# Gwzwpxz/HDSDP

Measured on AMD Instinct MI355X. Metric: IPM iterations/sec (Schur build+factor+solve), n=2000 m=2000 dense SDP, higher is better.
Workload: dtype f64

## Files before the change

### hdsdp_amd/csrc/chol.h

```cpp
#pragma once
#include "hdm_common.h"
#include <vector>

struct HdmChol {
    int n = 0, npad = 0, nblk = 0;
    HdmBuf<double> L;
    HdmBuf<double> Linv;
    HdmBuf<double> Dinv;
    HdmBuf<double> Z;
    HdmBuf<double> Zd;
    HdmBuf<double> vec;
    HdmBuf<int> info_dev;
    bool factored = false, have_inv = false;
    bool logdet_ok = false;
    double logdet_val = 0.0;
    HdmBuf<int> flow_flags;
    HdmPinned<int> flow_err;
    int flow_epoch = 0;
    bool flow_ok = true, flow_pending = false;
    int flow_cap = -1;
    std::vector<double> host_stage;
    std::vector<int> env_first, env_colh;
    HdmBuf<int> env_dev;
    HdmBuf<double> sgn;
    HdmBuf<int> sinfo_dev;

    int init(int n);
    int set_envelope(const int *first_blockcol_of_blockrow);
    int load_host(const double *A, long lda, hipStream_t s);
    int load_device(const double *A, long lda, hipStream_t s);
    int finish_load(hipStream_t s);
    int factor(hipStream_t s, int *info_host);
    int invert_factor(hipStream_t s);
    int set_reverse_inverse(hipStream_t s);
    int factor_signed(hipStream_t s, int *info_host, int *nneg_host);
    int reverse_signs(double *sig_dev, hipStream_t s);
    int get_diag(double *diag_host, hipStream_t s);
    int solve_device(double *b_dev, double *x_dev, int nrhs, long ldv, int which, hipStream_t s);
    int solve_host(const double *rhs, double *sol, int nrhs, int which, hipStream_t s);
    bool flow_gave_up();
    int inverse_full(double *out_dev, long ldo, hipStream_t s);
};

int hdm_potrf_sweep_configure();
int hdm_potrf_sweep_batched(double *tiles, const int *diag_tile, const int *cols, int ncols, double *Winv, int *info, int m, hipStream_t s,
                            double *sgn = nullptr);

void hdm_flow_set_shared_device(int on);
bool hdm_flow_shared_device();
double hdm_diag_block_probe(int variant, int reps, hipStream_t s);
```

### hdsdp_amd/csrc/chol.hip

```cpp
#include "hdm_common.h"
#include "chol.h"
#include "sweep128.h"
#include <algorithm>
#include <atomic>
#include <cstring>

#define NB 128

#define PB 32
#define LDW 98
__device__ __forceinline__ double hdm_readlane_f64(double v, int lane) {
    int lo = __double2loint(v), hi = __double2hiint(v);
    lo = __builtin_amdgcn_readlane(lo, lane);
    hi = __builtin_amdgcn_readlane(hi, lane);
    return __hiloint2double(hi, lo);
}

typedef double hdm_c4 __attribute__((ext_vector_type(4)));

template <int NT>
__device__ __forceinline__ void hdm_lds_mm(double *pc, int crs, int ccs, const double *pa, int ars, int acs, const double *pb,
                                           int brs, int bcs, int M, int N, int K, double alpha, int accumulate, int k_by_row,
                                           int lower_only, int wave, int lane, double *gout, long gld) {
    const int l15 = lane & 15, lq = lane >> 4;
    const int mt = M >> 4, nt = (N >> 4) / NT, units = mt * nt;
    for (int u = wave; u < units; u += 4) {
        const int ti = u / nt, tj = (u % nt) * NT;
        if (lower_only && tj > ti) continue;
        hdm_c4 acc[NT];
#pragma unroll
        for (int q = 0; q < NT; ++q) acc[q] = (hdm_c4){0.0, 0.0, 0.0, 0.0};
        const int kend = k_by_row ? min(K, (ti + 1) * 16) : K;
        const double *qa = pa + (ti * 16 + l15) * ars + lq * acs;
        const double *qb = pb + lq * brs + (tj * 16 + l15) * bcs;
        for (int k0 = 0; k0 < kend; k0 += 4) {
            const double av = qa[k0 * acs];
#pragma unroll
            for (int q = 0; q < NT; ++q) acc[q] = __builtin_amdgcn_mfma_f64_16x16x4f64(qb[k0 * brs + q * 16 * bcs], av, acc[q], 0, 0, 0);
        }
#pragma unroll
        for (int q = 0; q < NT; ++q)
#pragma unroll
            for (int r = 0; r < 4; ++r) {
                const int m = ti * 16 + l15, n = (tj + q) * 16 + lq + 4 * r;
                double *c = pc + m * crs + n * ccs;
                const double v = (accumulate ? *c : 0.0) + alpha * acc[q][r];
                *c = v;
                if (gout) gout[m + (long) n * gld] = v;
            }
    }
}

__global__ __launch_bounds__(256) void hdm_potrf_diag_kernel(double *__restrict__ A, long ld, double *__restrict__ Dinv,
                                                              int *__restrict__ info, int col0) {
    extern __shared__ __attribute__((aligned(16))) double sm[];
    double *a = sm;
    double *w = sm + NB * NB;
    const int tid = threadIdx.x;
    for (int e0 = tid; e0 < NB * NB; e0 += 256 * 16) {
        double v[16];
#pragma unroll
        for (int q = 0; q < 16; ++q) {
            const int e = e0 + q * 256;
            v[q] = A[(e & (NB - 1)) + (long) (e >> 7) * ld];
        }
#pragma unroll
        for (int q = 0; q < 16; ++q) {
            const int e = e0 + q * 256;
            a[e] = ((e & (NB - 1)) >= (e >> 7)) ? v[q] : 0.0;
        }
    }
    __syncthreads();

    for (int p = 0; p < NB / PB; ++p) {
        const int c0 = p * PB;
        if (tid < 64) {
            const int l = tid & 31;
            double *blk = a + c0 + c0 * NB;
            double row[PB], rinv[PB];
#pragma unroll
            for (int k = 0; k < PB; ++k) row[k] = blk[l + k * NB];
            int bad = 0;
#pragma unroll
            for (int j = 0; j < PB; ++j) {
                double d = hdm_readlane_f64(row[j], j);
                if (!(d > 0.0)) {
                    if (!bad) bad = j + 1;
                    d = 1.0;
                }
                const double piv = sqrt(d);
                double ri = 1.0 / piv;
                asm volatile("" : "+v"(ri));
                rinv[j] = ri;
                row[j] = (l == j) ? piv : row[j] * ri;
#pragma unroll
                for (int k = j + 1; k < PB; ++k) row[k] -= row[j] * hdm_readlane_f64(row[j], k);
                __builtin_amdgcn_sched_barrier(0);
            }
            if (bad && tid == 0) atomicCAS(info, 0, col0 + c0 + bad);
            if (tid < PB) {
#pragma unroll
                for (int k = 0; k < PB; ++k)
                    if (k <= l) A[(c0 + l) + (long) (c0 + k) * ld] = row[k];
            }
#pragma unroll
            for (int k = 0; k < PB; ++k) asm volatile("" : "+v"(row[k]));
            double x[PB];
#pragma unroll
            for (int i = 0; i < PB; ++i) {
                double sacc = (l == i) ? 1.0 : 0.0;
#pragma unroll
                for (int k = 0; k < i; ++k) sacc -= hdm_readlane_f64(row[k], i) * x[k];
                x[i] = (l <= i) ? sacc * rinv[i] : 0.0;
                __builtin_amdgcn_sched_barrier(0);
            }
            if (tid < PB) {
#pragma unroll
                for (int i = 0; i < PB; ++i) blk[i + l * NB] = x[i];
            }
        }
        __syncthreads();
        const int t0 = c0 + PB, nr = NB - t0;
        if (nr <= 0) break;
        const int wave = tid >> 6, lane = tid & 63;
        hdm_lds_mm<2>(a + t0 + c0 * NB, 1, NB, a + t0 + c0 * NB, 1, NB, a + c0 + c0 * NB, NB, 1, nr, PB, PB, 1.0, 0, 0, 0, wave,
                      lane, A + t0 + (long) c0 * ld, ld);
        __syncthreads();
        hdm_lds_mm<1>(a + t0 + t0 * NB, 1, NB, a + t0 + c0 * NB, 1, NB, a + t0 + c0 * NB, NB, 1, nr, nr, PB, -1.0, 1, 0, 1, wave,
                      lane, nullptr, 0);
        __syncthreads();
    }
    {
        const int wave = tid >> 6, lane = tid & 63;
        for (int j = NB / PB - 2; j >= 0; --j) {
            const int c0 = j * PB, r0 = c0 + PB, nr = NB - r0;
            hdm_lds_mm<2>(w, 1, LDW, a + r0 + c0 * NB, 1, NB, a + c0 + c0 * NB, 1, NB, nr, PB, PB, 1.0, 0, 0, 0, wave, lane,
                          nullptr, 0);
            __syncthreads();
            hdm_lds_mm<2>(a + r0 + c0 * NB, 1, NB, a + r0 + r0 * NB, 1, NB, w, 1, LDW, nr, PB, nr, -1.0, 0, 1, 0, wave, lane,
                          nullptr, 0);
            __syncthreads();
        }
    }
    for (int e = tid; e < NB * NB; e += 256) Dinv[e] = a[e];
}

#define DIAG_SWEEP_LDS_DOUBLES (SMALL_P * (SMALL_P + 1) + 2 * SMALL_P)
template <bool SIGNED = false>
__device__ __forceinline__ void hdm_potrf_diag_sweep_body(double *__restrict__ A, long ld, double *__restrict__ Dinv, int *__restrict__ info,
                                                          int col0, int nv, double *__restrict__ sgn_out = nullptr,
                                                          int *__restrict__ nneg_out = nullptr) {
    extern __shared__ __attribute__((aligned(16))) double sm[];
    double *img = sm;
    double *rsv = sm + SMALL_P * (SMALL_P + 1);
    constexpr int ldi = SMALL_P + 1;
    const int tid = threadIdx.x, ty = tid >> 5, tx = tid & 31;
    const int ei = tid & (SMALL_P - 1), ej0 = tid >> 7;
#pragma unroll 8
    for (int j = ej0; j < SMALL_P; j += SM_T / SMALL_P) img[ei + j * ldi] = (ei >= j) ? A[ei + (long) j * ld] : 0.0;
    __syncthreads();
    double a[SM_NR][SM_NC], rr[SM_NR][SM_NC];
#pragma unroll
    for (int r = 0; r < SM_NR; ++r)
#pragma unroll
        for (int c = 0; c < SM_NC; ++c) a[r][c] = img[(ty + 16 * r) + (tx + 32 * c) * ldi];
    __syncthreads();
    double unused;
    int nneg = 0;
    const int bad = sm_sweep<false, SIGNED>(nv, a, rr, img, rsv, ty, tx, &unused, &nneg);
    if (bad && tid == 0) atomicCAS(info, 0, col0 + bad);
    if (SIGNED) {
        if (tid < SMALL_P && sgn_out) sgn_out[tid] = (tid < nv && rsv[tid] < 0.0) ? -1.0 : 1.0;
        if (tid == 0 && nneg_out && nneg) atomicAdd(nneg_out, nneg);
    }
    __syncthreads();
    sm_store_one<true>(SMALL_P, a, img, A, ld, ty, tx, tid);
    sm_store_one<false>(SMALL_P, rr, img, Dinv, SMALL_P, ty, tx, tid);
}
__global__ __launch_bounds__(SM_T) void hdm_potrf_diag_sweep_kernel(double *__restrict__ A, long ld, double *__restrict__ Dinv,
                                                                    int *__restrict__ info, int col0, int nv) {
    hdm_potrf_diag_sweep_body(A, ld, Dinv, info, col0, nv);
}
__global__ __launch_bounds__(SM_T) void hdm_potrf_diag_sweep_signed_kernel(double *__restrict__ A, long ld, double *__restrict__ Dinv,
                                                                           int *__restrict__ info, int col0, int nv,
                                                                           double *__restrict__ sgn) {
    hdm_potrf_diag_sweep_body<true>(A, ld, Dinv, info, col0, nv, sgn, info + 1);
}
template <bool SIGNED>
__global__ __launch_bounds__(SM_T) void hdm_potrf_diag_sweep_tiles_kernel(double *__restrict__ tiles, const int *__restrict__ diag_tile,
                                                                          const int *__restrict__ cols, double *__restrict__ Winv,
                                                                          int *__restrict__ info, int m, double *__restrict__ sgn) {
    const int k = cols[blockIdx.x];
    int dummy = 0;
    (void) dummy;
    double *A = tiles + ((long) diag_tile[k] << 14);
    __shared__ int linfo;
    if (threadIdx.x == 0) linfo = 0;
    __syncthreads();
    hdm_potrf_diag_sweep_body<SIGNED>(A, SMALL_P, Winv + ((long) k << 14), &linfo, k * SMALL_P, min(SMALL_P, m - k * SMALL_P),
                                      SIGNED ? sgn + (long) k * SMALL_P : nullptr, SIGNED ? info + 1 : nullptr);
    __syncthreads();
    if (threadIdx.x == 0 && linfo) {
        int old = atomicCAS(info, 0, linfo);
        while (old != 0 && linfo < old) { const int seen = atomicCAS(info, old, linfo); if (seen == old) break; old = seen; }
    }
}
int hdm_potrf_sweep_configure() {
    HDM_HIP_CHECK(hipFuncSetAttribute((const void *) hdm_potrf_diag_sweep_tiles_kernel<false>, hipFuncAttributeMaxDynamicSharedMemorySize,
                                      DIAG_SWEEP_LDS_DOUBLES * (int) sizeof(double)));
    HDM_HIP_CHECK(hipFuncSetAttribute((const void *) hdm_potrf_diag_sweep_tiles_kernel<true>, hipFuncAttributeMaxDynamicSharedMemorySize,
                                      DIAG_SWEEP_LDS_DOUBLES * (int) sizeof(double)));
    return 0;
}
int hdm_potrf_sweep_batched(double *tiles, const int *diag_tile, const int *cols, int ncols, double *Winv, int *info, int m, hipStream_t s,
                            double *sgn) {
    if (ncols <= 0) return 0;
    if (sgn)
        hipLaunchKernelGGL(hdm_potrf_diag_sweep_tiles_kernel<true>, dim3(ncols), dim3(SM_T), DIAG_SWEEP_LDS_DOUBLES * sizeof(double), s, tiles,
                           diag_tile, cols, Winv, info, m, sgn);
    else
        hipLaunchKernelGGL(hdm_potrf_diag_sweep_tiles_kernel<false>, dim3(ncols), dim3(SM_T), DIAG_SWEEP_LDS_DOUBLES * sizeof(double), s, tiles,
                           diag_tile, cols, Winv, info, m, sgn);
    HDM_HIP_CHECK(hipGetLastError());
    return 0;
}

__global__ void hdm_pad_identity_kernel(double *A, long ld, int n, int npad) {
    long e = (long) blockIdx.x * blockDim.x + threadIdx.x;
    long tot = (long) npad * npad;
    if (e >= tot) return;
    int i = (int) (e % npad), j = (int) (e / npad);
    if (i >= n || j >= n) A[i + (long) j * ld] = (i == j) ? 1.0 : 0.0;
}

__global__ void hdm_reverse_factor_kernel(const double *__restrict__ F, double *__restrict__ W, long ld, int n, int npad) {
    long e = (long) blockIdx.x * blockDim.x + threadIdx.x;
    long tot = (long) npad * npad;
    if (e >= tot) return;
    int i = (int) (e % npad), j = (int) (e / npad);
    double v;
    if (i >= n || j >= n) v = (i == j) ? 1.0 : 0.0;
    else v = (i >= j) ? F[(n - 1 - j) + (long) (n - 1 - i) * ld] : 0.0;
    W[i + (long) j * ld] = v;
}

__global__ void hdm_signed_panel_kernel(double *__restrict__ P, long ld, double *__restrict__ Z, long ldz,
                                        const double *__restrict__ sg, int rows) {
    const long e = (long) blockIdx.x * blockDim.x + threadIdx.x;
    if (e >= (long) rows * NB) return;
    const int i = (int) (e % rows), j = (int) (e / rows);
    const double q = P[i + (long) j * ld];
    Z[i + (long) j * ldz] = q;
    P[i + (long) j * ld] = q * sg[j];
}
__global__ void hdm_reverse_signs_kernel(const double *__restrict__ sgn, double *__restrict__ sig, int n, int npad) {
    const int i = blockIdx.x * blockDim.x + threadIdx.x;
    if (i < npad) sig[i] = (i < n) ? sgn[n - 1 - i] : 1.0;
}
__global__ void hdm_zero_words_kernel(int *p, int count) { if ((int) threadIdx.x < count) p[threadIdx.x] = 0; }

__global__ void hdm_copy_diag_blocks_kernel(const double *__restrict__ Dinv, double *__restrict__ Linv, long ld) {
    const int e = blockIdx.x * 256 + threadIdx.x, k = blockIdx.y;
    Linv[(long) k * NB * (ld + 1) + (e & (NB - 1)) + (long) (e >> 7) * ld] = Dinv[(long) k * NB * NB + e];
}

__global__ void hdm_copy_block_kernel(const double *__restrict__ src, long lds_, double *__restrict__ dst, long ldd,
                                      int rows, int cols) {
    long e = (long) blockIdx.x * blockDim.x + threadIdx.x;
    if (e >= (long) rows * cols) return;
    int i = (int) (e % rows), j = (int) (e / rows);
    dst[i + (long) j * ldd] = src[i + (long) j * lds_];
}

__global__ void hdm_get_diag_kernel(const double *__restrict__ A, long ld, int n, double *__restrict__ d) {
    int i = blockIdx.x * blockDim.x + threadIdx.x;
    if (i < n) d[i] = A[i + (long) i * ld];
}

__global__ __launch_bounds__(256) void hdm_trsv_fwd_step(const double *__restrict__ L, long ld,
                                                          const double *__restrict__ Dinv, double *__restrict__ b,
                                                          double *__restrict__ x, int k, int nblk, int nrhs, long ldv) {
    __shared__ double yk[NB];
    __shared__ double part[256];
    const int tid = threadIdx.x;
    const int bi = k + blockIdx.x;
    const int rhs = blockIdx.y;
    double *bb = b + (long) rhs * ldv, *xx = x + (long) rhs * ldv;
    const double *D = Dinv + (long) k * NB * NB;
    {
        int r = tid & (NB - 1), h = tid >> 7;
        double s = 0.0;
        for (int c = h; c <= r; c += 2) s += D[r + c * NB] * bb[k * NB + c];
        part[tid] = s;
        __syncthreads();
        if (tid < NB) yk[tid] = part[tid] + part[tid + NB];
        __syncthreads();
    }
    if (bi == k) {
        if (tid < NB) xx[k * NB + tid] = yk[tid];
        return;
    }
    if (bi >= nblk) return;
    {
        int r = tid & (NB - 1), h = tid >> 7;
        const double *Lb = L + (long) bi * NB + (long) k * NB * ld;
        double s = 0.0;
        for (int c = h * 64; c < h * 64 + 64; ++c) s += Lb[r + (long) c * ld] * yk[c];
        part[tid] = s;
        __syncthreads();
        if (tid < NB) bb[bi * NB + tid] -= part[tid] + part[tid + NB];
    }
}

__global__ __launch_bounds__(256) void hdm_trsv_bwd_step(const double *__restrict__ L, long ld,
                                                          const double *__restrict__ Dinv, double *__restrict__ y,
                                                          double *__restrict__ x, int k, int nrhs, long ldv) {
    __shared__ double xk[NB];
    __shared__ double part[256];
    const int tid = threadIdx.x;
    const int bi = (int) blockIdx.x;
    const int rhs = blockIdx.y;
    double *yy = y + (long) rhs * ldv, *xx = x + (long) rhs * ldv;
    const double *D = Dinv + (long) k * NB * NB;
    {
        int c = tid & (NB - 1), h = tid >> 7;
        double s = 0.0;
        for (int r = c + h; r < NB; r += 2) s += D[r + c * NB] * yy[k * NB + r];
        part[tid] = s;
        __syncthreads();
        if (tid < NB) xk[tid] = part[tid] + part[tid + NB];
        __syncthreads();
    }
    if (bi == k) {
        if (tid < NB) xx[k * NB + tid] = xk[tid];
        return;
    }
    {
        const double *Lb = L + (long) k * NB + (long) bi * NB * ld;
        const int lane = tid & 63, wave = tid >> 6;
        for (int cc = 0; cc < 32; ++cc) {
            int c = wave * 32 + cc;
            double s = Lb[lane + (long) c * ld] * xk[lane] + Lb[lane + 64 + (long) c * ld] * xk[lane + 64];
            for (int off = 32; off > 0; off >>= 1) s += __shfl_down(s, off, 64);
            if (lane == 0) yy[bi * NB + c] -= s;
        }
    }
}

__device__ __forceinline__ bool hdm_flow_wait(const int *flag, int epoch) {
    for (int it = 0; it < (1 << 22); ++it) {
        if (__hip_atomic_load(flag, __ATOMIC_ACQUIRE, __HIP_MEMORY_SCOPE_AGENT) == epoch) return true;
        __builtin_amdgcn_s_sleep(2);
    }
    return false;
}

__device__ __forceinline__ double hdm_row_dot_half(const double *__restrict__ Mb, long ld, const double *v, int tid) {
    const int r = tid & (NB - 1), h = tid >> 7;
    const double *q = Mb + r + (long) (h * 64) * ld;
    double s0 = 0.0, s1 = 0.0;
#pragma unroll 16
    for (int c = 0; c < 64; c += 2) {
        s0 += q[(long) c * ld] * v[h * 64 + c];
        s1 += q[(long) (c + 1) * ld] * v[h * 64 + c + 1];
    }
    return s0 + s1;
}
template <bool SUBTRACT>
__device__ __forceinline__ void hdm_col_dots(const double *__restrict__ Mb, long ld, const double *v, double *out, int wave,
                                             int lane) {
    const double v0 = v[lane], v1 = v[lane + 64];
    for (int cc = 0; cc < 32; cc += 8) {
        double sacc[8];
#pragma unroll
        for (int q = 0; q < 8; ++q) {
            const double *col = Mb + (long) (wave * 32 + cc + q) * ld;
            sacc[q] = col[lane] * v0 + col[lane + 64] * v1;
        }
#pragma unroll
        for (int off = 32; off > 0; off >>= 1)
#pragma unroll
            for (int q = 0; q < 8; ++q) sacc[q] += __shfl_down(sacc[q], off, 64);
        if (lane == 0) {
#pragma unroll
            for (int q = 0; q < 8; ++q) {
                if (SUBTRACT) out[wave * 32 + cc + q] -= sacc[q];
                else out[wave * 32 + cc + q] = sacc[q];
            }
        }
    }
}

__global__ __launch_bounds__(256) void hdm_trsv_flow_kernel(const double *__restrict__ L, long ld,
                                                             const double *__restrict__ Dinv, const double *b, double *y,
                                                             double *x, int nblk, long ldv, int *flags, int epoch,
                                                             int which, volatile int *err, const int *__restrict__ env) {
    __shared__ double v[NB];
    __shared__ double acc[NB];
    __shared__ double part[256];
    __shared__ int ok;
    const int tid = threadIdx.x, lane = tid & 63, wave = tid >> 6;
    const int i = blockIdx.x, rhs = blockIdx.y;
    const double *bb = b + (long) rhs * ldv;
    double *yy = y + (long) rhs * ldv, *xx = x + (long) rhs * ldv;
    int *ff = flags + (long) rhs * 2 * nblk, *fb = ff + nblk;
    const double *D = Dinv + (long) i * NB * NB;
    if (tid < NB) acc[tid] = bb[i * NB + tid];
    if (tid == 0) ok = 1;
    __syncthreads();
    const int kfirst = env ? env[i] : 0, klast = env ? env[nblk + i] : nblk - 1;
    if (which != 2) {
        for (int k = kfirst; k < i; ++k) {
            if (tid == 0 && !hdm_flow_wait(ff + k, epoch)) ok = 0;
            __syncthreads();
            if (!ok) { if (tid == 0) *err = 1; return; }
            __builtin_amdgcn_fence(__ATOMIC_ACQUIRE, "agent");
            if (tid < NB) v[tid] = __builtin_nontemporal_load(yy + k * NB + tid);
            __syncthreads();
            part[tid] = hdm_row_dot_half(L + (long) i * NB + (long) k * NB * ld, ld, v, tid);
            __syncthreads();
            if (tid < NB) acc[tid] -= part[tid] + part[tid + NB];
            __syncthreads();
        }
        part[tid] = hdm_row_dot_half(D, NB, acc, tid);
        __syncthreads();
        if (tid < NB) {
            const double val = part[tid] + part[tid + NB];
            acc[tid] = val;
            yy[i * NB + tid] = val;
            if (which == 1) xx[i * NB + tid] = val;
        }
        __threadfence();
        __syncthreads();
        if (tid == 0) __hip_atomic_store(ff + i, epoch, __ATOMIC_RELEASE, __HIP_MEMORY_SCOPE_AGENT);
        if (which == 1) return;
    }
    for (int k = klast; k > i; --k) {
        if (tid == 0 && !hdm_flow_wait(fb + k, epoch)) ok = 0;
        __syncthreads();
        if (!ok) { if (tid == 0) *err = 1; return; }
        __builtin_amdgcn_fence(__ATOMIC_ACQUIRE, "agent");
        if (tid < NB) v[tid] = __builtin_nontemporal_load(xx + k * NB + tid);
        __syncthreads();
        hdm_col_dots<true>(L + (long) k * NB + (long) i * NB * ld, ld, v, acc, wave, lane);
        __syncthreads();
    }
    hdm_col_dots<false>(D, NB, acc, part, wave, lane);
    __syncthreads();
    if (tid < NB) xx[i * NB + tid] = part[tid];
    __threadfence();
    __syncthreads();
    if (tid == 0) __hip_atomic_store(fb + i, epoch, __ATOMIC_RELEASE, __HIP_MEMORY_SCOPE_AGENT);
}

__global__ void hdm_probe_spd_block_kernel(double *A, long ld) {
    const int e = blockIdx.x * blockDim.x + threadIdx.x;
    const int i = e & (NB - 1), j = e >> 7;
    if (j < NB) A[i + (long) j * ld] = (i == j) ? 4.0 + 0.01 * i : 1.0 / (1.0 + abs(i - j));
}
double hdm_diag_block_probe(int variant, int reps, hipStream_t s) {
    HdmBuf<double> A_own, D_own;
    HdmBuf<int> info_own;
    hipEvent_t e0, e1;
    if (A_own.alloc(NB * NB) != hipSuccess || D_own.alloc(NB * NB) != hipSuccess ||
        info_own.alloc(1) != hipSuccess || hipEventCreate(&e0) != hipSuccess || hipEventCreate(&e1) != hipSuccess)
        return -1.0;
    double *A = A_own.get(), *D = D_own.get();
    int *info = info_own.get();
    (void) hipFuncSetAttribute((const void *) hdm_potrf_diag_kernel, hipFuncAttributeMaxDynamicSharedMemorySize, (NB * NB + LDW * PB) * (int) sizeof(double));
    (void) hipFuncSetAttribute((const void *) hdm_potrf_diag_sweep_kernel, hipFuncAttributeMaxDynamicSharedMemorySize, DIAG_SWEEP_LDS_DOUBLES * (int) sizeof(double));
    (void) hipMemsetAsync(info, 0, sizeof(int), s);
    float ms = 0.f, total = 0.f;
    for (int r = -2; r < reps; ++r) {
        hipLaunchKernelGGL(hdm_probe_spd_block_kernel, dim3(NB * NB / 256), dim3(256), 0, s, A, (long) NB);
        (void) hipEventRecord(e0, s);
        if (variant)
            hipLaunchKernelGGL(hdm_potrf_diag_sweep_kernel, dim3(1), dim3(SM_T), DIAG_SWEEP_LDS_DOUBLES * sizeof(double), s, A, (long) NB, D, info, 0, NB);
        else
            hipLaunchKernelGGL(hdm_potrf_diag_kernel, dim3(1), dim3(256), (NB * NB + LDW * PB) * sizeof(double), s, A, (long) NB, D, info, 0);
        (void) hipEventRecord(e1, s);
        (void) hipEventSynchronize(e1);
        (void) hipEventElapsedTime(&ms, e0, e1);
        if (r >= 0) total += ms;
    }
    (void) hipEventDestroy(e0); (void) hipEventDestroy(e1);
    return total / reps * 1e3;
}

int HdmChol::init(int n_) {
    n = n_;
    npad = (int) hdm_roundup(n, NB);
    nblk = npad / NB;
    size_t mat = sizeof(double) * (size_t) npad * npad;
    HDM_HIP_CHECK(L.alloc((size_t) npad * npad));
    HDM_HIP_CHECK(Dinv.alloc((size_t) nblk * NB * NB));
    HDM_HIP_CHECK(info_dev.alloc(1));
    HDM_HIP_CHECK(vec.alloc((size_t) npad * 4));
    HDM_HIP_CHECK(hdm_memset_sync(L.get(), 0, mat));
    HDM_HIP_CHECK(hipFuncSetAttribute((const void *) hdm_potrf_diag_kernel, hipFuncAttributeMaxDynamicSharedMemorySize,
                                      (NB * NB + LDW * PB) * (int) sizeof(double)));
    HDM_HIP_CHECK(hipFuncSetAttribute((const void *) hdm_potrf_diag_sweep_kernel, hipFuncAttributeMaxDynamicSharedMemorySize,
                                      DIAG_SWEEP_LDS_DOUBLES * (int) sizeof(double)));
    return 0;
}

int HdmChol::set_envelope(const int *first) {
    env_first.clear(); env_colh.clear();
    env_dev.reset();
    if (!first || nblk <= 1) return 0;
    env_first.assign(first, first + nblk);
    env_colh.assign(nblk, 0);
    for (int i = 0; i < nblk; ++i) {
        env_first[i] = std::max(0, std::min(env_first[i], i));
        if (i > 0) env_first[i] = std::min(env_first[i], i);
    }
    for (int k = 0; k < nblk; ++k) env_colh[k] = k;
    for (int i = 0; i < nblk; ++i)
        for (int k = env_first[i]; k <= i; ++k) env_colh[k] = std::max(env_colh[k], i);
    for (int k = 1; k < nblk; ++k) env_colh[k] = std::max(env_colh[k], env_colh[k - 1]);
    std::vector<int> both(env_first);
    both.insert(both.end(), env_colh.begin(), env_colh.end());
    HDM_HIP_CHECK(env_dev.alloc(both.size()));
    HDM_HIP_CHECK(hdm_memcpy_h2d_sync(env_dev.get(), both.data(), sizeof(int) * both.size()));
    return 0;
}

int HdmChol::load_host(const double *A, long lda, hipStream_t s) {
    HDM_HIP_CHECK(hipMemcpy2DAsync(L.get(), sizeof(double) * npad, A, sizeof(double) * lda, sizeof(double) * n, n,
                                   hipMemcpyHostToDevice, s));
    return finish_load(s);
}

int HdmChol::load_device(const double *A, long lda, hipStream_t s) {
    HDM_HIP_CHECK(hipMemcpy2DAsync(L.get(), sizeof(double) * npad, A, sizeof(double) * lda, sizeof(double) * n, n,
                                   hipMemcpyDeviceToDevice, s));
    return finish_load(s);
}

int HdmChol::finish_load(hipStream_t s) {
    if (npad != n) {
        long tot = (long) npad * npad;
        hipLaunchKernelGGL(hdm_pad_identity_kernel, dim3((unsigned) ((tot + 255) / 256)), dim3(256), 0, s, L.get(),
                           (long) npad, n, npad);
        HDM_HIP_CHECK(hipGetLastError());
    }
    factored = false;
    have_inv = false;
    logdet_ok = false;
    return 0;
}

int HdmChol::set_reverse_inverse(hipStream_t s) {
    if (!factored) return 1;
    HDM_HIP_CHECK(Linv.reserve((size_t) npad * npad));
    long tot = (long) npad * npad;
    hipLaunchKernelGGL(hdm_reverse_factor_kernel, dim3((unsigned) ((tot + 255) / 256)), dim3(256), 0, s, L.get(), Linv.get(),
                       (long) npad, n, npad);
    HDM_HIP_CHECK(hipGetLastError());
    have_inv = true;
    return 0;
}

typedef unsigned hdm_k2 __attribute__((ext_vector_type(2)));
template <int NJ, bool UPDATE>
__global__ __launch_bounds__(256) void hdm_k128_kernel(const double *__restrict__ A, long lda, const double *__restrict__ B, long ldb,
                                                       double *C, long ldc) {
    constexpr int KB = (NJ == 2) ? 8 : 4;
    const int ti = blockIdx.x, tj = blockIdx.y;
    if (UPDATE && ti < tj) return;
    const int tid = threadIdx.x, lane = tid & 63;
    const int wave = __builtin_amdgcn_readfirstlane(tid >> 6);
    const int l15 = lane & 15, lq = lane >> 4;
    const int r0 = ti * 64 + (wave & 1) * 32, c0 = tj * (32 * NJ) + (wave >> 1) * (16 * NJ);
    const __amdgpu_buffer_rsrc_t ra = __builtin_amdgcn_make_buffer_rsrc(const_cast<double *>(A + r0), 0, 0x7fffffff, 0x00020000);
    const __amdgpu_buffer_rsrc_t rb = __builtin_amdgcn_make_buffer_rsrc(const_cast<double *>(B + c0), 0, 0x7fffffff, 0x00020000);
    const unsigned va = (unsigned) ((l15 + lq * lda) * 8), vb = (unsigned) ((l15 + lq * ldb) * 8);
    const unsigned sa = (unsigned) (4 * lda * 8), sb = (unsigned) (4 * ldb * 8);
    hdm_c4 acc[NJ][2];
#pragma unroll
    for (int j = 0; j < NJ; ++j)
#pragma unroll
        for (int i = 0; i < 2; ++i) acc[j][i] = (hdm_c4){0.0, 0.0, 0.0, 0.0};
    hdm_k2 fa[2][KB][NJ], fb[2][KB][2];
#define K128_LOAD(SET, BLK)                                                                                      \
    _Pragma("unroll") for (int q = 0; q < KB; ++q) {                                                             \
        _Pragma("unroll") for (int i = 0; i < 2; ++i)                                                            \
            fb[SET][q][i] = __builtin_amdgcn_raw_buffer_load_b64(ra, va + 128 * i, ((BLK) * KB + q) * sa, 0);    \
        _Pragma("unroll") for (int j = 0; j < NJ; ++j)                                                           \
            fa[SET][q][j] = __builtin_amdgcn_raw_buffer_load_b64(rb, vb + 128 * j, ((BLK) * KB + q) * sb, 0);    \
    }
#define K128_MMA(SET)                                                                                            \
    _Pragma("unroll") for (int q = 0; q < KB; ++q)                                                               \
        _Pragma("unroll") for (int j = 0; j < NJ; ++j)                                                           \
            _Pragma("unroll") for (int i = 0; i < 2; ++i)                                                        \
                acc[j][i] = __builtin_amdgcn_mfma_f64_16x16x4f64(__builtin_bit_cast(double, fa[SET][q][j]),      \
                                                                 __builtin_bit_cast(double, fb[SET][q][i]), acc[j][i], 0, 0, 0);
    constexpr int NBLK = 32 / KB;
    K128_LOAD(0, 0) K128_LOAD(1, 1)
#pragma unroll
    for (int b = 0; b < NBLK; b += 2) {
        K128_MMA(0)
        if (b + 2 < NBLK) { K128_LOAD(0, b + 2) }
        K128_MMA(1)
        if (b + 3 < NBLK) { K128_LOAD(1, b + 3) }
    }
#undef K128_LOAD
#undef K128_MMA
    if (!UPDATE) __syncthreads();
    double *cl = C + (r0 + l15) + (long) (c0 + lq) * ldc;
    const bool diag = UPDATE && (ti == tj);
#pragma unroll
    for (int j = 0; j < NJ; ++j)
#pragma unroll
        for (int r = 0; r < 4; ++r)
#pragma unroll
            for (int i = 0; i < 2; ++i) {
                double *q = cl + 16 * i + (long) (16 * j + 4 * r) * ldc;
                if (UPDATE) {
                    if (diag && (r0 + 16 * i + l15) < (c0 + 16 * j + lq + 4 * r)) continue;
                    *q = -1.0 * acc[j][i][r] + 1.0 * (*q);
                } else {
                    *q = 1.0 * acc[j][i][r];
                }
            }
}

static int hdm_k128_launch(bool update, const double *A, long lda, const double *B, long ldb, double *C, long ldc, int rows,
                           hipStream_t s) {
    if (update) hipLaunchKernelGGL((hdm_k128_kernel<2, true>), dim3(rows / 64, rows / 64), dim3(256), 0, s, A, lda, B, ldb, C, ldc);
    else hipLaunchKernelGGL((hdm_k128_kernel<4, false>), dim3(rows / 64, 1), dim3(256), 0, s, A, lda, B, ldb, C, ldc);
    HDM_HIP_CHECK(hipGetLastError());
    return 0;
}

static bool hdm_chol_k128(int rows, long ld) {
    return hdm_env_on<ENV_CHOL_K128>() && rows % 64 == 0 && ld < (1L << 20);
}
static int hdm_chol_panel(double *P, long ld, const double *Dk, int rows, hipStream_t s) {
    if (hdm_chol_k128(rows, ld)) return hdm_k128_launch(false, P, ld, Dk, NB, P, ld, rows, s);
    return hdm_launch_gemm(hdm_gemm_product(P, ld, rows, NB, NB, 1.0, hdm_mmajor(P, ld), hdm_mmajor(Dk, NB)), s);
}
static int hdm_chol_update(double *A22, long ld, const double *P, const double *Q, long ldq, int rows, hipStream_t s) {
    if (hdm_chol_k128(rows, ld)) return hdm_k128_launch(true, P, ld, Q, ldq, A22, ld, rows, s);
    return hdm_launch_gemm(hdm_gemm_product(A22, ld, rows, rows, NB, -1.0, hdm_mmajor(P, ld), hdm_mmajor(Q, ldq), 1.0, hdm_lower()), s);
}

__global__ void hdm_zero_word_kernel(int *p) { *p = 0; }

int HdmChol::factor(hipStream_t s, int *info_host) {
    hipLaunchKernelGGL(hdm_zero_word_kernel, dim3(1), dim3(1), 0, s, info_dev.get());
    HDM_HIP_CHECK(hipGetLastError());
    const long ld = npad;
    const size_t shm = (NB * NB + LDW * PB) * sizeof(double);
    const bool diag_sweep = hdm_env_on<ENV_DIAG_SWEEP>();
    for (int k = 0; k < nblk; ++k) {
        double *Akk = L.get() + (long) k * NB * (ld + 1);
        if (diag_sweep)
            hipLaunchKernelGGL(hdm_potrf_diag_sweep_kernel, dim3(1), dim3(SM_T), DIAG_SWEEP_LDS_DOUBLES * sizeof(double), s, Akk, ld,
                               Dinv.get() + (long) k * NB * NB, info_dev.get(), k * NB, std::max(1, std::min(NB, n - k * NB)));
        else
            hipLaunchKernelGGL(hdm_potrf_diag_kernel, dim3(1), dim3(256), shm, s, Akk, ld, Dinv.get() + (long) k * NB * NB,
                               info_dev.get(), k * NB);
        HDM_HIP_CHECK(hipGetLastError());
        if (npad - (k + 1) * NB <= 0) break;
        const int rows = env_colh.empty() ? npad - (k + 1) * NB : (env_colh[k] - k) * NB;
        if (rows <= 0) continue;
        double *P = Akk + NB;
        if (hdm_chol_panel(P, ld, Dinv.get() + (long) k * NB * NB, rows, s)) return 1;
        if (hdm_chol_update(Akk + (long) NB * (ld + 1), ld, P, P, ld, rows, s)) return 1;
    }
    int info = 0;
    HDM_HIP_CHECK(hipMemcpyAsync(&info, info_dev.get(), sizeof(int), hipMemcpyDeviceToHost, s));
    HDM_HIP_CHECK(hipStreamSynchronize(s));
    if (info > n) info = 0;
    if (info_host) *info_host = info;
    factored = (info == 0);
    have_inv = false;
    return 0;
}

int HdmChol::factor_signed(hipStream_t s, int *info_host, int *nneg_host) {
    if (!sgn.get()) {
        HDM_HIP_CHECK(sgn.alloc((size_t) npad));
        HDM_HIP_CHECK(sinfo_dev.alloc(2));
        HDM_HIP_CHECK(hipFuncSetAttribute((const void *) hdm_potrf_diag_sweep_signed_kernel, hipFuncAttributeMaxDynamicSharedMemorySize,
                                          DIAG_SWEEP_LDS_DOUBLES * (int) sizeof(double)));
    }
    if (!Z.get() && nblk > 1) HDM_HIP_CHECK(Z.alloc((size_t) npad * NB));
    hipLaunchKernelGGL(hdm_zero_words_kernel, dim3(1), dim3(64), 0, s, sinfo_dev.get(), 2);
    HDM_HIP_CHECK(hipGetLastError());
    const long ld = npad;
    for (int k = 0; k < nblk; ++k) {
        double *Akk = L.get() + (long) k * NB * (ld + 1);
        hipLaunchKernelGGL(hdm_potrf_diag_sweep_signed_kernel, dim3(1), dim3(SM_T), DIAG_SWEEP_LDS_DOUBLES * sizeof(double), s, Akk, ld,
                           Dinv.get() + (long) k * NB * NB, sinfo_dev.get(), k * NB, std::max(1, std::min(NB, n - k * NB)), sgn.get() + (long) k * NB);
        HDM_HIP_CHECK(hipGetLastError());
        const int rows = npad - (k + 1) * NB;
        if (rows <= 0) break;
        double *P = Akk + NB;
        if (hdm_chol_panel(P, ld, Dinv.get() + (long) k * NB * NB, rows, s)) return 1;
        const long tot = (long) rows * NB;
        hipLaunchKernelGGL(hdm_signed_panel_kernel, dim3((unsigned) ((tot + 255) / 256)), dim3(256), 0, s, P, ld, Z.get(), (long) npad,
                           (const double *) (sgn.get() + (long) k * NB), rows);
        HDM_HIP_CHECK(hipGetLastError());
        if (hdm_chol_update(Akk + (long) NB * (ld + 1), ld, P, Z.get(), npad, rows, s)) return 1;
    }
    int info[2] = {0, 0};
    HDM_HIP_CHECK(hipMemcpyAsync(info, sinfo_dev.get(), sizeof(int) * 2, hipMemcpyDeviceToHost, s));
    HDM_HIP_CHECK(hipStreamSynchronize(s));
    if (info[0] > n) info[0] = 0;
    if (info_host) *info_host = info[0];
    if (nneg_host) *nneg_host = info[1];
    factored = (info[0] == 0);
    have_inv = false;
    logdet_ok = false;
    return 0;
}

int HdmChol::reverse_signs(double *sig_dev, hipStream_t s) {
    if (!sgn.get() || !factored) return 1;
    hipLaunchKernelGGL(hdm_reverse_signs_kernel, dim3((npad + 255) / 256), dim3(256), 0, s, (const double *) sgn.get(), sig_dev, n, npad);
    HDM_HIP_CHECK(hipGetLastError());
    return 0;
}

int HdmChol::invert_factor(hipStream_t s) {
    if (have_inv) return 0;
    const long ld = npad;
    size_t mat = sizeof(double) * (size_t) npad * npad;
    HDM_HIP_CHECK(Linv.reserve(mat / sizeof(double)));
    if (!Z.get() && nblk > 1) HDM_HIP_CHECK(Z.alloc((size_t) npad * NB));
    HDM_HIP_CHECK(hipMemsetAsync(Linv.get(), 0, mat, s));
    if (nblk >= 2 && (nblk & (nblk - 1)) == 0) {
        HDM_HIP_CHECK(Zd.reserve(mat / sizeof(double)));
        hipLaunchKernelGGL(hdm_copy_diag_blocks_kernel, dim3(NB * NB / 256, nblk), dim3(256), 0, s, Dinv.get(), Linv.get(), ld);
        HDM_HIP_CHECK(hipGetLastError());
        for (long sz = NB; sz < npad; sz *= 2) {
            const int pairs = (int) (npad / (2 * sz));
            const long pstride = 2 * sz * (ld + 1);
            const int m = (int) sz;
            if (hdm_launch_gemm(hdm_gemm_product(Zd.get() + sz, ld, m, m, m, 1.0, hdm_mmajor(L.get() + sz, ld, pstride), hdm_kmajor(Linv.get(), ld, pstride),
                                                 0.0, hdm_batched(pairs, pstride)), s)) return 1;
            if (hdm_launch_gemm(hdm_gemm_product(Linv.get() + sz, ld, m, m, m, -1.0, hdm_mmajor(Linv.get() + sz * (ld + 1), ld, pstride),
                                                 hdm_kmajor(Zd.get() + sz, ld, pstride), 0.0, hdm_klimit(HDM_KLIM_BY_M).batched(pairs, pstride)), s)) return 1;
        }
        have_inv = true;
        return 0;
    }
    for (int k = nblk - 1; k >= 0; --k) {
        double *Xkk = Linv.get() + (long) k * NB * (ld + 1);
        hipLaunchKernelGGL(hdm_copy_block_kernel, dim3(NB * NB / 256), dim3(256), 0, s, Dinv.get() + (long) k * NB * NB,
                           (long) NB, Xkk, ld, NB, NB);
        HDM_HIP_CHECK(hipGetLastError());
        const int rows = npad - (k + 1) * NB;
        if (rows <= 0) continue;
        const double *P = L.get() + (long) k * NB * (ld + 1) + NB;
        if (hdm_launch_gemm(hdm_gemm_product(Z.get(), npad, rows, NB, NB, 1.0, hdm_mmajor(P, ld), hdm_kmajor(Dinv.get() + (long) k * NB * NB, NB)), s)) return 1;
        if (hdm_launch_gemm(hdm_gemm_product(Xkk + NB, ld, rows, NB, rows, -1.0, hdm_mmajor(Linv.get() + (long) (k + 1) * NB * (ld + 1), ld),
                                             hdm_kmajor(Z.get(), npad), 0.0, hdm_klimit(HDM_KLIM_BY_M)), s)) return 1;
    }
    have_inv = true;
    return 0;
}

int HdmChol::get_diag(double *diag_host, hipStream_t s) {
    hipLaunchKernelGGL(hdm_get_diag_kernel, dim3((n + 255) / 256), dim3(256), 0, s, L.get(), (long) npad, n, vec.get());
    HDM_HIP_CHECK(hipGetLastError());
    HDM_HIP_CHECK(hipMemcpyAsync(diag_host, vec.get(), sizeof(double) * n, hipMemcpyDeviceToHost, s));
    HDM_HIP_CHECK(hipStreamSynchronize(s));
    return 0;
}

static std::atomic<int> g_flow_shared_device{0};
void hdm_flow_set_shared_device(int on) { g_flow_shared_device.store(on); }
bool hdm_flow_shared_device() { return g_flow_shared_device.load() != 0; }
static bool hdm_flow_enabled() { return hdm_env_on<ENV_TRSV_FLOW>() && g_flow_shared_device.load() == 0; }

int HdmChol::solve_device(double *b_dev, double *x_dev, int nrhs, long ldv, int which, hipStream_t s) {
    const long ld = npad;
    if (flow_cap < 0) {
        int dev = 0, cus = 0, per_cu = 0;
        if (hipGetDevice(&dev) == hipSuccess &&
            hipDeviceGetAttribute(&cus, hipDeviceAttributeMultiprocessorCount, dev) == hipSuccess &&
            hipOccupancyMaxActiveBlocksPerMultiprocessor(&per_cu, hdm_trsv_flow_kernel, 256, 0) == hipSuccess)
            flow_cap = cus * std::max(1, per_cu);
        else
            flow_cap = 0;
        (void) hipGetLastError();
    }
    if (hdm_flow_enabled() && flow_ok && nrhs <= 2 && (long) nblk * nrhs <= flow_cap) {
        if (!flow_flags) {
            HDM_HIP_CHECK(flow_flags.alloc(4 * (size_t) nblk));
            HDM_HIP_CHECK(hdm_memset_sync(flow_flags.get(), 0, sizeof(int) * 4 * (size_t) nblk));
            HDM_HIP_CHECK(flow_err.alloc(1, hipHostMallocMapped));
            *flow_err.get() = 0;
        }
        int *err_dev = flow_err.dev();
        ++flow_epoch;
        hipLaunchKernelGGL(hdm_trsv_flow_kernel, dim3(nblk, nrhs), dim3(256), 0, s, L.get(), ld, Dinv.get(), b_dev, b_dev, x_dev, nblk,
                           ldv, flow_flags.get(), flow_epoch, which, err_dev, (const int *) env_dev.get());
        HDM_HIP_CHECK(hipGetLastError());
        flow_pending = true;
        return 0;
    }
    double *cur = b_dev;
    if (which == 0 || which == 1) {
        for (int k = 0; k < nblk; ++k) {
            hipLaunchKernelGGL(hdm_trsv_fwd_step, dim3(nblk - k, nrhs), dim3(256), 0, s, L.get(), ld, Dinv.get(), cur, x_dev, k,
                               nblk, nrhs, ldv);
        }
        HDM_HIP_CHECK(hipGetLastError());
        if (which == 1) return 0;
        HDM_HIP_CHECK(hipMemcpyAsync(cur, x_dev, sizeof(double) * ldv * nrhs, hipMemcpyDeviceToDevice, s));
    }
    for (int k = nblk - 1; k >= 0; --k) {
        hipLaunchKernelGGL(hdm_trsv_bwd_step, dim3(k + 1, nrhs), dim3(256), 0, s, L.get(), ld, Dinv.get(), cur, x_dev, k, nrhs,
                           ldv);
    }
    HDM_HIP_CHECK(hipGetLastError());
    return 0;
}

static bool hdm_flow_fail_once() {
    static bool left = hdm_env_on<ENV_TRSV_FLOW_FAIL_ONCE>();
    if (left) { left = false; return true; }
    return false;
}

bool HdmChol::flow_gave_up() {
    bool gave_up = flow_pending && flow_err && *(volatile int *) flow_err.get() != 0;
    if (flow_pending && hdm_flow_fail_once()) gave_up = true;
    flow_pending = false;
    if (gave_up) {
        fprintf(stderr, "[hdsdp_mi355x] single-launch substitution timed out; using per-block launches\n");
        flow_ok = false;
        if (flow_err) *flow_err.get() = 0;
    }
    return gave_up;
}

int HdmChol::solve_host(const double *rhs, double *sol, int nrhs, int which, hipStream_t s) {
    const int chunk = 2;
    if (host_stage.size() < (size_t) chunk * n) host_stage.resize((size_t) chunk * n);
    for (int c0 = 0; c0 < nrhs; c0 += chunk) {
        int nc = (nrhs - c0 < chunk) ? nrhs - c0 : chunk;
        double *b = vec.get(), *x = vec.get() + 2L * npad;
        HDM_HIP_CHECK(hipMemsetAsync(vec.get(), 0, sizeof(double) * 4L * npad, s));
        HDM_HIP_CHECK(hipMemcpy2DAsync(b, sizeof(double) * npad, rhs + (long) c0 * n, sizeof(double) * n,
                                       sizeof(double) * n, nc, hipMemcpyHostToDevice, s));
        if (solve_device(b, x, nc, npad, which, s)) return 1;
        HDM_HIP_CHECK(hipMemcpy2DAsync(host_stage.data(), sizeof(double) * n, x, sizeof(double) * npad,
                                       sizeof(double) * n, nc, hipMemcpyDeviceToHost, s));
        HDM_HIP_CHECK(hipStreamSynchronize(s));
        if (flow_gave_up()) {
            c0 -= chunk;
            continue;
        }
        memcpy(sol + (long) c0 * n, host_stage.data(), sizeof(double) * (size_t) n * nc);
    }
    return 0;
}

int HdmChol::inverse_full(double *out_dev, long ldo, hipStream_t s) {
    if (invert_factor(s)) return 1;
    const HdmOperand Lt = hdm_kmajor(Linv.get(), npad);
    return hdm_launch_gemm(hdm_gemm_product(out_dev, ldo, npad, npad, npad, 1.0, Lt, Lt), s);
}

const void *hdm_module_handle_chol() { return (const void *) hdm_potrf_diag_kernel; }
```

Before: 2.893.

## Prefetch L tiles into registers in flow TRSV and add lookahead trailing-update stream

The dataflow triangular-solve kernel now double-buffers the next 128x128 L tile in registers while it waits on the dependency flag for the current one. It also stages the diagonal inverse block into dynamic LDS at kernel start, so memory latency overlaps the inter-block waits. Separately, the Cholesky trailing update is split so the first block column runs on the main stream and the rest runs on a side stream joined after the next diagonal factor. That lookahead only activates for matrices with at least 4096 trailing rows. The cost is heavy register use (two 64-double arrays per thread) plus 128KB of LDS per block, which lowers occupancy and the flow capacity check.

After: 2.890. About the same (-0.1%).

```diff
diff --git a/hdsdp_amd/csrc/chol.h b/hdsdp_amd/csrc/chol.h
--- a/hdsdp_amd/csrc/chol.h
+++ b/hdsdp_amd/csrc/chol.h
@@ -1,6 +1,22 @@
 #pragma once
 #include "hdm_common.h"
 #include <vector>
+
+struct HdmSideStream {
+    hipStream_t s = nullptr;
+    std::vector<hipEvent_t> fork, done;
+    HdmSideStream() = default;
+    HdmSideStream(const HdmSideStream &) = delete;
+    HdmSideStream &operator=(const HdmSideStream &) = delete;
+    HdmSideStream(HdmSideStream &&o) noexcept : s(o.s), fork(std::move(o.fork)), done(std::move(o.done)) { o.s = nullptr; o.fork.clear(); o.done.clear(); }
+    HdmSideStream &operator=(HdmSideStream &&o) noexcept {
+        if (this != &o) { reset(); s = o.s; fork = std::move(o.fork); done = std::move(o.done); o.s = nullptr; o.fork.clear(); o.done.clear(); }
+        return *this;
+    }
+    ~HdmSideStream() { reset(); }
+    void reset();
+    hipError_t create(int nevents);
+};
 
 struct HdmChol {
     int n = 0, npad = 0, nblk = 0;
@@ -24,6 +40,8 @@
     HdmBuf<int> env_dev;
     HdmBuf<double> sgn;
     HdmBuf<int> sinfo_dev;
+    HdmSideStream side;
+    int side_pending = -1;
 
     int init(int n);
     int set_envelope(const int *first_blockcol_of_blockrow);
@@ -40,6 +58,8 @@
     int solve_host(const double *rhs, double *sol, int nrhs, int which, hipStream_t s);
     bool flow_gave_up();
     int inverse_full(double *out_dev, long ldo, hipStream_t s);
+    int trailing_update(int k, double *A22, const double *P, const double *Q, long ldq, int rows, hipStream_t s);
+    int side_join(hipStream_t s);
 };
 
 int hdm_potrf_sweep_configure();
diff --git a/hdsdp_amd/csrc/chol.hip b/hdsdp_amd/csrc/chol.hip
--- a/hdsdp_amd/csrc/chol.hip
+++ b/hdsdp_amd/csrc/chol.hip
@@ -391,10 +391,54 @@
     }
 }
 
+__device__ __forceinline__ void hdm_flow_fetch_rows(double (&o)[64], const double *__restrict__ Mb, long ld, int tid) {
+    const double *q = Mb + (tid & (NB - 1)) + (long) ((tid >> 7) * 64) * ld;
+#pragma unroll
+    for (int c = 0; c < 64; ++c) o[c] = q[(long) c * ld];
+}
+__device__ __forceinline__ void hdm_flow_fetch_cols(double (&o)[64], const double *__restrict__ Mb, long ld, int wave, int lane) {
+#pragma unroll
+    for (int c = 0; c < 32; ++c) {
+        const double *col = Mb + (long) (wave * 32 + c) * ld;
+        o[2 * c] = col[lane];
+        o[2 * c + 1] = col[lane + 64];
+    }
+}
+__device__ __forceinline__ double hdm_row_dot_held(const double (&o)[64], const double *v, int tid) {
+    const int h = tid >> 7;
+    double s0 = 0.0, s1 = 0.0;
+#pragma unroll
+    for (int c = 0; c < 64; c += 2) {
+        s0 += o[c] * v[h * 64 + c];
+        s1 += o[c + 1] * v[h * 64 + c + 1];
+    }
+    return s0 + s1;
+}
+__device__ __forceinline__ void hdm_col_dots_held(const double (&o)[64], const double *v, double *out, int wave, int lane) {
+    const double v0 = v[lane], v1 = v[lane + 64];
+#pragma unroll
+    for (int cc = 0; cc < 32; cc += 8) {
+        double sacc[8];
+#pragma unroll
+        for (int q = 0; q < 8; ++q) sacc[q] = o[2 * (cc + q)] * v0 + o[2 * (cc + q) + 1] * v1;
+#pragma unroll
+        for (int off = 32; off > 0; off >>= 1)
+#pragma unroll
+            for (int q = 0; q < 8; ++q) sacc[q] += __shfl_down(sacc[q], off, 64);
+        if (lane == 0) {
+#pragma unroll
+            for (int q = 0; q < 8; ++q) out[wave * 32 + cc + q] -= sacc[q];
+        }
+    }
+}
+
+#define HDM_FLOW_LDS_BYTES (NB * NB * (int) sizeof(double))
+#define HDM_AHEAD_MIN_ROWS 4096
 __global__ __launch_bounds__(256) void hdm_trsv_flow_kernel(const double *__restrict__ L, long ld,
                                                              const double *__restrict__ Dinv, const double *b, double *y,
                                                              double *x, int nblk, long ldv, int *flags, int epoch,
                                                              int which, volatile int *err, const int *__restrict__ env) {
+    extern __shared__ __attribute__((aligned(16))) double Dl[];
     __shared__ double v[NB];
     __shared__ double acc[NB];
     __shared__ double part[256];
@@ -404,25 +448,56 @@
     const double *bb = b + (long) rhs * ldv;
     double *yy = y + (long) rhs * ldv, *xx = x + (long) rhs * ldv;
     int *ff = flags + (long) rhs * 2 * nblk, *fb = ff + nblk;
-    const double *D = Dinv + (long) i * NB * NB;
-    if (tid < NB) acc[tid] = bb[i * NB + tid];
+    const int kfirst = env ? env[i] : 0, klast = env ? env[nblk + i] : nblk - 1;
+    const double *Lrow = L + (long) i * NB, *Lcol = L + (long) i * NB * ld;
+    double op0[64], op1[64];
+    if (which != 2) {
+        if (kfirst < i) hdm_flow_fetch_rows(op0, Lrow + (long) kfirst * NB * ld, ld, tid);
+    } else if (klast > i) {
+        hdm_flow_fetch_cols(op0, Lcol + (long) klast * NB, ld, wave, lane);
+    }
+    {
+        const double *D = Dinv + (long) i * NB * NB;
+        for (int e0 = tid; e0 < NB * NB; e0 += 256 * 32) {
+            double d[32];
+#pragma unroll
+            for (int q = 0; q < 32; ++q) d[q] = D[e0 + q * 256];
+#pragma unroll
+            for (int q = 0; q < 32; ++q) Dl[e0 + q * 256] = d[q];
+        }
+    }
+    double a = 0.0;
+    if (tid < NB) {
+        a = bb[i * NB + tid];
+        if (which == 2) acc[tid] = a;
+    }
     if (tid == 0) ok = 1;
     __syncthreads();
-    const int kfirst = env ? env[i] : 0, klast = env ? env[nblk + i] : nblk - 1;
     if (which != 2) {
-        for (int k = kfirst; k < i; ++k) {
+        auto step = [&](const double (&o)[64], int k) -> bool {
             if (tid == 0 && !hdm_flow_wait(ff + k, epoch)) ok = 0;
             __syncthreads();
-            if (!ok) { if (tid == 0) *err = 1; return; }
+            if (!ok) { if (tid == 0) *err = 1; return false; }
             __builtin_amdgcn_fence(__ATOMIC_ACQUIRE, "agent");
             if (tid < NB) v[tid] = __builtin_nontemporal_load(yy + k * NB + tid);
             __syncthreads();
-            part[tid] = hdm_row_dot_half(L + (long) i * NB + (long) k * NB * ld, ld, v, tid);
+            part[tid] = hdm_row_dot_held(o, v, tid);
             __syncthreads();
-            if (tid < NB) acc[tid] -= part[tid] + part[tid + NB];
-            __syncthreads();
-        }
-        part[tid] = hdm_row_dot_half(D, NB, acc, tid);
+            if (tid < NB) a -= part[tid] + part[tid + NB];
+            return true;
+        };
+        for (int k = kfirst; k < i;) {
+            if (k + 1 < i) hdm_flow_fetch_rows(op1, Lrow + (long) (k + 1) * NB * ld, ld, tid);
+            if (!step(op0, k)) return;
+            if (++k >= i) break;
+            if (k + 1 < i) hdm_flow_fetch_rows(op0, Lrow + (long) (k + 1) * NB * ld, ld, tid);
+            if (!step(op1, k)) return;
+            ++k;
+        }
+        if (which == 0 && klast > i) hdm_flow_fetch_cols(op0, Lcol + (long) klast * NB, ld, wave, lane);
+        if (tid < NB) acc[tid] = a;
+        __syncthreads();
+        part[tid] = hdm_row_dot_half(Dl, NB, acc, tid);
         __syncthreads();
         if (tid < NB) {
             const double val = part[tid] + part[tid + NB];
@@ -435,17 +510,28 @@
         if (tid == 0) __hip_atomic_store(ff + i, epoch, __ATOMIC_RELEASE, __HIP_MEMORY_SCOPE_AGENT);
         if (which == 1) return;
     }
-    for (int k = klast; k > i; --k) {
-        if (tid == 0 && !hdm_flow_wait(fb + k, epoch)) ok = 0;
-        __syncthreads();
-        if (!ok) { if (tid == 0) *err = 1; return; }
-        __builtin_amdgcn_fence(__ATOMIC_ACQUIRE, "agent");
-        if (tid < NB) v[tid] = __builtin_nontemporal_load(xx + k * NB + tid);
-        __syncthreads();
-        hdm_col_dots<true>(L + (long) k * NB + (long) i * NB * ld, ld, v, acc, wave, lane);
-        __syncthreads();
-    }
-    hdm_col_dots<false>(D, NB, acc, part, wave, lane);
+    {
+        auto step = [&](const double (&o)[64], int k) -> bool {
+            if (tid == 0 && !hdm_flow_wait(fb + k, epoch)) ok = 0;
+            __syncthreads();
+            if (!ok) { if (tid == 0) *err = 1; return false; }
+            __builtin_amdgcn_fence(__ATOMIC_ACQUIRE, "agent");
+            if (tid < NB) v[tid] = __builtin_nontemporal_load(xx + k * NB + tid);
+            __syncthreads();
+            hdm_col_dots_held(o, v, acc, wave, lane);
+            __syncthreads();
+            return true;
+        };
+        for (int k = klast; k > i;) {
+            if (k - 1 > i) hdm_flow_fetch_cols(op1, Lcol + (long) (k - 1) * NB, ld, wave, lane);
+            if (!step(op0, k)) return;
+            if (--k <= i) break;
+            if (k - 1 > i) hdm_flow_fetch_cols(op0, Lcol + (long) (k - 1) * NB, ld, wave, lane);
+            if (!step(op1, k)) return;
+            --k;
+        }
+    }
+    hdm_col_dots<false>(Dl, NB, acc, part, wave, lane);
     __syncthreads();
     if (tid < NB) xx[i * NB + tid] = part[tid];
     __threadfence();
@@ -501,6 +587,10 @@
                                       (NB * NB + LDW * PB) * (int) sizeof(double)));
     HDM_HIP_CHECK(hipFuncSetAttribute((const void *) hdm_potrf_diag_sweep_kernel, hipFuncAttributeMaxDynamicSharedMemorySize,
                                       DIAG_SWEEP_LDS_DOUBLES * (int) sizeof(double)));
+    HDM_HIP_CHECK(hipFuncSetAttribute((const void *) hdm_trsv_flow_kernel, hipFuncAttributeMaxDynamicSharedMemorySize, HDM_FLOW_LDS_BYTES));
+    side.reset();
+    side_pending = -1;
+    if (npad - NB >= HDM_AHEAD_MIN_ROWS) HDM_HIP_CHECK(side.create(nblk));
     return 0;
 }
 
@@ -564,9 +654,9 @@
 typedef unsigned hdm_k2 __attribute__((ext_vector_type(2)));
 template <int NJ, bool UPDATE>
 __global__ __launch_bounds__(256) void hdm_k128_kernel(const double *__restrict__ A, long lda, const double *__restrict__ B, long ldb,
-                                                       double *C, long ldc) {
+                                                       double *C, long ldc, int ti0) {
     constexpr int KB = (NJ == 2) ? 8 : 4;
-    const int ti = blockIdx.x, tj = blockIdx.y;
+    const int ti = blockIdx.x + ti0, tj = blockIdx.y;
     if (UPDATE && ti < tj) return;
     const int tid = threadIdx.x, lane = tid & 63;
     const int wave = __builtin_amdgcn_readfirstlane(tid >> 6);
@@ -626,9 +716,9 @@
 }
 
 static int hdm_k128_launch(bool update, const double *A, long lda, const double *B, long ldb, double *C, long ldc, int rows,
-                           hipStream_t s) {
-    if (update) hipLaunchKernelGGL((hdm_k128_kernel<2, true>), dim3(rows / 64, rows / 64), dim3(256), 0, s, A, lda, B, ldb, C, ldc);
-    else hipLaunchKernelGGL((hdm_k128_kernel<4, false>), dim3(rows / 64, 1), dim3(256), 0, s, A, lda, B, ldb, C, ldc);
+                           hipStream_t s, int row0 = 0) {
+    if (update) hipLaunchKernelGGL((hdm_k128_kernel<2, true>), dim3((rows - row0) / 64, rows / 64), dim3(256), 0, s, A, lda, B, ldb, C, ldc, row0 / 64);
+    else hipLaunchKernelGGL((hdm_k128_kernel<4, false>), dim3(rows / 64, 1), dim3(256), 0, s, A, lda, B, ldb, C, ldc, 0);
     HDM_HIP_CHECK(hipGetLastError());
     return 0;
 }
@@ -640,12 +730,51 @@
     if (hdm_chol_k128(rows, ld)) return hdm_k128_launch(false, P, ld, Dk, NB, P, ld, rows, s);
     return hdm_launch_gemm(hdm_gemm_product(P, ld, rows, NB, NB, 1.0, hdm_mmajor(P, ld), hdm_mmajor(Dk, NB)), s);
 }
-static int hdm_chol_update(double *A22, long ld, const double *P, const double *Q, long ldq, int rows, hipStream_t s) {
-    if (hdm_chol_k128(rows, ld)) return hdm_k128_launch(true, P, ld, Q, ldq, A22, ld, rows, s);
+static int hdm_chol_update(double *A22, long ld, const double *P, const double *Q, long ldq, int rows, hipStream_t s, int row0 = 0) {
+    if (hdm_chol_k128(rows, ld)) return hdm_k128_launch(true, P, ld, Q, ldq, A22, ld, rows, s, row0);
+    if (row0) return 1;
     return hdm_launch_gemm(hdm_gemm_product(A22, ld, rows, rows, NB, -1.0, hdm_mmajor(P, ld), hdm_mmajor(Q, ldq), 1.0, hdm_lower()), s);
 }
 
 __global__ void hdm_zero_word_kernel(int *p) { *p = 0; }
+
+void HdmSideStream::reset() {
+    for (hipEvent_t e : fork) if (e) (void) hipEventDestroy(e);
+    for (hipEvent_t e : done) if (e) (void) hipEventDestroy(e);
+    fork.clear(); done.clear();
+    if (s) (void) hipStreamDestroy(s);
+    s = nullptr;
+}
+hipError_t HdmSideStream::create(int nevents) {
+    reset();
+    hipError_t e = hipStreamCreateWithFlags(&s, hipStreamNonBlocking);
+    if (e != hipSuccess) { s = nullptr; return e; }
+    fork.assign(nevents, nullptr); done.assign(nevents, nullptr);
+    for (int k = 0; k < nevents && e == hipSuccess; ++k) {
+        e = hipEventCreateWithFlags(&fork[k], hipEventDisableTiming);
+        if (e == hipSuccess) e = hipEventCreateWithFlags(&done[k], hipEventDisableTiming);
+    }
+    if (e != hipSuccess) reset();
+    return e;
+}
+
+int HdmChol::trailing_update(int k, double *A22, const double *P, const double *Q, long ldq, int rows, hipStream_t s) {
+    const long ld = npad;
+    if (!side.s || rows < HDM_AHEAD_MIN_ROWS || !hdm_chol_k128(rows, ld)) return hdm_chol_update(A22, ld, P, Q, ldq, rows, s);
+    if (hdm_chol_update(A22, ld, P, Q, ldq, NB, s)) return 1;
+    HDM_HIP_CHECK(hipEventRecord(side.fork[k], s));
+    HDM_HIP_CHECK(hipStreamWaitEvent(side.s, side.fork[k], 0));
+    if (hdm_chol_update(A22, ld, P, Q, ldq, rows, side.s, NB)) return 1;
+    HDM_HIP_CHECK(hipEventRecord(side.done[k], side.s));
+    side_pending = k;
+    return 0;
+}
+int HdmChol::side_join(hipStream_t s) {
+    if (side_pending < 0) return 0;
+    HDM_HIP_CHECK(hipStreamWaitEvent(s, side.done[side_pending], 0));
+    side_pending = -1;
+    return 0;
+}
 
 int HdmChol::factor(hipStream_t s, int *info_host) {
     hipLaunchKernelGGL(hdm_zero_word_kernel, dim3(1), dim3(1), 0, s, info_dev.get());
@@ -662,13 +791,15 @@
             hipLaunchKernelGGL(hdm_potrf_diag_kernel, dim3(1), dim3(256), shm, s, Akk, ld, Dinv.get() + (long) k * NB * NB,
                                info_dev.get(), k * NB);
         HDM_HIP_CHECK(hipGetLastError());
+        if (side_join(s)) return 1;
         if (npad - (k + 1) * NB <= 0) break;
         const int rows = env_colh.empty() ? npad - (k + 1) * NB : (env_colh[k] - k) * NB;
         if (rows <= 0) continue;
         double *P = Akk + NB;
         if (hdm_chol_panel(P, ld, Dinv.get() + (long) k * NB * NB, rows, s)) return 1;
-        if (hdm_chol_update(Akk + (long) NB * (ld + 1), ld, P, P, ld, rows, s)) return 1;
-    }
+        if (trailing_update(k, Akk + (long) NB * (ld + 1), P, P, ld, rows, s)) return 1;
+    }
+    if (side_join(s)) return 1;
     int info = 0;
     HDM_HIP_CHECK(hipMemcpyAsync(&info, info_dev.get(), sizeof(int), hipMemcpyDeviceToHost, s));
     HDM_HIP_CHECK(hipStreamSynchronize(s));
@@ -695,6 +826,7 @@
         hipLaunchKernelGGL(hdm_potrf_diag_sweep_signed_kernel, dim3(1), dim3(SM_T), DIAG_SWEEP_LDS_DOUBLES * sizeof(double), s, Akk, ld,
                            Dinv.get() + (long) k * NB * NB, sinfo_dev.get(), k * NB, std::max(1, std::min(NB, n - k * NB)), sgn.get() + (long) k * NB);
         HDM_HIP_CHECK(hipGetLastError());
+        if (side_join(s)) return 1;
         const int rows = npad - (k + 1) * NB;
         if (rows <= 0) break;
         double *P = Akk + NB;
@@ -703,8 +835,9 @@
         hipLaunchKernelGGL(hdm_signed_panel_kernel, dim3((unsigned) ((tot + 255) / 256)), dim3(256), 0, s, P, ld, Z.get(), (long) npad,
                            (const double *) (sgn.get() + (long) k * NB), rows);
         HDM_HIP_CHECK(hipGetLastError());
-        if (hdm_chol_update(Akk + (long) NB * (ld + 1), ld, P, Z.get(), npad, rows, s)) return 1;
-    }
+        if (trailing_update(k, Akk + (long) NB * (ld + 1), P, Z.get(), npad, rows, s)) return 1;
+    }
+    if (side_join(s)) return 1;
     int info[2] = {0, 0};
     HDM_HIP_CHECK(hipMemcpyAsync(info, sinfo_dev.get(), sizeof(int) * 2, hipMemcpyDeviceToHost, s));
     HDM_HIP_CHECK(hipStreamSynchronize(s));
@@ -782,7 +915,7 @@
         int dev = 0, cus = 0, per_cu = 0;
         if (hipGetDevice(&dev) == hipSuccess &&
             hipDeviceGetAttribute(&cus, hipDeviceAttributeMultiprocessorCount, dev) == hipSuccess &&
-            hipOccupancyMaxActiveBlocksPerMultiprocessor(&per_cu, hdm_trsv_flow_kernel, 256, 0) == hipSuccess)
+            hipOccupancyMaxActiveBlocksPerMultiprocessor(&per_cu, hdm_trsv_flow_kernel, 256, HDM_FLOW_LDS_BYTES) == hipSuccess)
             flow_cap = cus * std::max(1, per_cu);
         else
             flow_cap = 0;
@@ -797,7 +930,7 @@
         }
         int *err_dev = flow_err.dev();
         ++flow_epoch;
-        hipLaunchKernelGGL(hdm_trsv_flow_kernel, dim3(nblk, nrhs), dim3(256), 0, s, L.get(), ld, Dinv.get(), b_dev, b_dev, x_dev, nblk,
+        hipLaunchKernelGGL(hdm_trsv_flow_kernel, dim3(nblk, nrhs), dim3(256), HDM_FLOW_LDS_BYTES, s, L.get(), ld, Dinv.get(), b_dev, b_dev, x_dev, nblk,
                            ldv, flow_flags.get(), flow_epoch, which, err_dev, (const int *) env_dev.get());
         HDM_HIP_CHECK(hipGetLastError());
         flow_pending = true;
```
